# zhvng/open-musiclm

Measured on NVIDIA H100. Metric: coarse-stage training tokens/sec (positions fed to the transformer per optimiser step / step time), higher is better.
Workload: dtype bf16 (fp16 operands for the forward GEMMs on LayerNorm outputs x weights; fp32 accumulate)

## Files before the change

### open-musiclm_b200/csrc/gemm_tc.cu

```cuda
#include "common.cuh"
#include "ptx.cuh"
#include "../../include/omlm_b200.h"
#include <stdlib.h>
#include <algorithm>

namespace omlm {

constexpr int BM = 128;
constexpr int BK = 64;
constexpr int kGemmThreads = 384;

struct EpiParams {
  void* out;
  const float* addend;
  long ldo;
  long ldadd;
  float alpha;
  int out_f32;
  int atomic;
  long split_stride;
  int vec_ok;
  int row_split;
  int row_valid;
  int n_valid;
  const __nv_bfloat16* rs_hn;
  long rs_ldhn;
  const float* rs_gamma;
  const uint8_t* rs_keep;
  float2* rs_part;
  float rs_keep_scale;
  int rs_parts;
};

__device__ __forceinline__ float bf16lo(uint32_t v) { return __uint_as_float(v << 16); }
__device__ __forceinline__ float bf16hi(uint32_t v) { return __uint_as_float(v & 0xffff0000u); }

template <int BN>
struct GemmSmem {
  static constexpr int kABytes = BM * BK * 2;
  static constexpr int kBBytes = BN * BK * 2;
  static constexpr int kStageBytes = kABytes + kBBytes;
  static constexpr int kMaxStages = 8;
};

template <int BN, int A_MN, int B_MN, bool F16, bool RS = false>
__global__ void __launch_bounds__(kGemmThreads, 1)
gemm_bf16_kernel(const __grid_constant__ CUtensorMap tmA, const __grid_constant__ CUtensorMap tmB,
                 const EpiParams ep, const int M, const int N, const int K, const int splits, const int kStages) {
  using S = GemmSmem<BN>;
  extern __shared__ uint8_t smem_raw[];
  uint8_t* smem = smem_raw + ((1024u - (smem_u32(smem_raw) & 1023u)) & 1023u);
  uint64_t* full_bar = reinterpret_cast<uint64_t*>(smem + kStages * S::kStageBytes);
  uint64_t* empty_bar = full_bar + S::kMaxStages;

  const int wg = threadIdx.x >> 7;
  const int lane = threadIdx.x & 31;

  const int m_tiles = (M + BM - 1) / BM;
  const int n_tiles = (N + BN - 1) / BN;
  const int kb_total = (K + BK - 1) / BK;
  const int kb_per_split = (kb_total + splits - 1) / splits;
  const int tiles_total = m_tiles * n_tiles;
  const int work_total = tiles_total * splits;

  if (threadIdx.x == 0) {
    tma_prefetch_desc(&tmA);
    tma_prefetch_desc(&tmB);
    for (int i = 0; i < kStages; ++i) {
      mbar_init(&full_bar[i], 1);
      mbar_init(&empty_bar[i], 2);
    }
    fence_barrier_init();
  }
  __syncthreads();

  if (wg == 0) {
    asm volatile("setmaxnreg.dec.sync.aligned.u32 40;");
    if (threadIdx.x == 0) {
      int stage = 0;
      uint32_t phase = 0;
      for (int w = blockIdx.x; w < work_total; w += gridDim.x) {
        const int split = w / tiles_total;
        const int tile = w - split * tiles_total;
        const int n_blk = tile % n_tiles, m_blk = tile / n_tiles;
        const int kb0 = split * kb_per_split;
        const int kb1 = min(kb_total, kb0 + kb_per_split);
        for (int kb = kb0; kb < kb1; ++kb) {
          mbar_wait(&empty_bar[stage], phase ^ 1);
          uint8_t* sa = smem + stage * S::kStageBytes;
          uint8_t* sb = sa + S::kABytes;
          mbar_expect_tx(&full_bar[stage], S::kStageBytes);
          if (A_MN == 0) {
            tma_load_2d(sa, &tmA, &full_bar[stage], kb * BK, m_blk * BM);
          } else {
#pragma unroll
            for (int c = 0; c < BM / 64; ++c)
              tma_load_2d(sa + c * 8192, &tmA, &full_bar[stage], m_blk * BM + c * 64, kb * BK);
          }
          if (B_MN == 0) {
            tma_load_2d(sb, &tmB, &full_bar[stage], kb * BK, n_blk * BN);
          } else {
#pragma unroll
            for (int c = 0; c < BN / 64; ++c)
              tma_load_2d(sb + c * 8192, &tmB, &full_bar[stage], n_blk * BN + c * 64, kb * BK);
          }
          if (++stage == kStages) { stage = 0; phase ^= 1; }
        }
      }
    }
    return;
  }

  asm volatile("setmaxnreg.inc.sync.aligned.u32 232;");
  const int cw = wg - 1;
  const int wq = (threadIdx.x >> 5) & 3;
  const int qr = lane >> 2, qc = lane & 3;
  const bool leader = (threadIdx.x & 127) == 0;
  int stage = 0;
  uint32_t phase = 0;
  for (int w = blockIdx.x; w < work_total; w += gridDim.x) {
    const int split = w / tiles_total;
    const int tile = w - split * tiles_total;
    const int n_blk = tile % n_tiles, m_blk = tile / n_tiles;
    const int kb0 = split * kb_per_split;
    const int kb1 = min(kb_total, kb0 + kb_per_split);
    float acc[BN / 2];
#pragma unroll
    for (int i = 0; i < BN / 2; ++i) acc[i] = 0.f;
    int prev = -1;
    for (int kb = kb0; kb < kb1; ++kb) {
      mbar_wait(&full_bar[stage], phase);
      const uint32_t sa = smem_u32(smem + stage * S::kStageBytes) + cw * 8192;
      const uint32_t sb = smem_u32(smem + stage * S::kStageBytes + S::kABytes);
      wgmma_fence();
#pragma unroll
      for (int k = 0; k < BK / 16; ++k) {
        const uint64_t ad = A_MN ? make_smem_desc(sa + k * 2048, 8192, 1024) : make_smem_desc(sa + k * 32, 16, 1024);
        const uint64_t bd = B_MN ? make_smem_desc(sb + k * 2048, 8192, 1024) : make_smem_desc(sb + k * 32, 16, 1024);
        const uint32_t accum = (kb > kb0 || k > 0) ? 1u : 0u;
        Wgmma<BN, F16>::template ss<A_MN, B_MN>(acc, ad, bd, accum);
      }
      wgmma_commit();
      wgmma_wait<1>();
      if (prev >= 0 && leader) mbar_arrive(&empty_bar[prev]);
      prev = stage;
      if (++stage == kStages) { stage = 0; phase ^= 1; }
    }
    wgmma_wait<0>();
    wgmma_reg_fence(acc);
    if (prev >= 0 && leader) mbar_arrive(&empty_bar[prev]);

    int row_in[2];
    long orow[2], arow[2];
    bool row_ok[2];
#pragma unroll
    for (int hr = 0; hr < 2; ++hr) {
      int row = m_blk * BM + cw * 64 + wq * 16 + qr + hr * 8;
      row_in[hr] = row;
      row_ok[hr] = row < M;
      if (ep.row_split > 0) {
        const int half = row / ep.row_split, r = row - half * ep.row_split;
        row_ok[hr] = row_ok[hr] && r < ep.row_valid;
        row = half * ep.row_valid + r;
      } else if (ep.row_split < 0) {
        const int w256 = row & 255, ch = ((row >> 8) << 7) + (w256 & 127);
        row_ok[hr] = row_ok[hr] && ch < ep.row_valid;
        row = (w256 >> 7) * ep.row_valid + ch;
      }
      orow[hr] = static_cast<long>(row) * ep.ldo;
      arow[hr] = static_cast<long>(row) * ep.ldadd;
    }
    constexpr int kEpiBatch = RS ? 4 : 8;
    float rs1[2][2] = {{0.f, 0.f}, {0.f, 0.f}}, rs2[2][2] = {{0.f, 0.f}, {0.f, 0.f}};
#pragma unroll
    for (int i0 = 0; i0 < BN / 8; i0 += kEpiBatch) {
      float2 add[2][kEpiBatch], gam[kEpiBatch];
      uint32_t hv[2][kEpiBatch], keep[2][kEpiBatch];
#pragma unroll
      for (int j = 0; j < kEpiBatch; ++j) {
        const int col = n_blk * BN + 8 * (i0 + j) + 2 * qc;
        const bool c0_ok = col < ep.n_valid, c1_ok = col + 1 < ep.n_valid;
        if constexpr (RS) gam[j] = c0_ok ? __ldg(reinterpret_cast<const float2*>(ep.rs_gamma + col)) : make_float2(0.f, 0.f);
#pragma unroll
// ... 32 lines not shown
            rs2[hr][hf] = fmaf(v0, bf16lo(hv[hr][j]), rs2[hr][hf]);
            rs2[hr][hf] = fmaf(v1, bf16hi(hv[hr][j]), rs2[hr][hf]);
          }
          if (!RS && ep.addend != nullptr) { v0 += add[hr][j].x; v1 += add[hr][j].y; }
          if (ep.atomic) {
            float* op = reinterpret_cast<float*>(ep.out) + orow[hr] + col;
            if (pair) asm volatile("red.global.add.v2.f32 [%0], {%1, %2};" ::"l"(op), "f"(v0), "f"(v1) : "memory");
            else { atomicAdd(op, v0); if (col + 1 < ep.n_valid) atomicAdd(op + 1, v1); }
          } else if (ep.out_f32) {
            float* op = reinterpret_cast<float*>(ep.out) + split * ep.split_stride + orow[hr] + col;
            if (pair) *reinterpret_cast<float2*>(op) = make_float2(v0, v1);
            else { op[0] = v0; if (col + 1 < ep.n_valid) op[1] = v1; }
          } else {
            __nv_bfloat16* op = reinterpret_cast<__nv_bfloat16*>(ep.out) + orow[hr] + col;
            if (pair) *reinterpret_cast<uint32_t*>(op) = pack_bf16x2(v0, v1);
            else { op[0] = __float2bfloat16_rn(v0); if (col + 1 < ep.n_valid) op[1] = __float2bfloat16_rn(v1); }
          }
        }
      }
    }
    if constexpr (RS) {
#pragma unroll
      for (int hr = 0; hr < 2; ++hr)
#pragma unroll
        for (int hf = 0; hf < 2; ++hf) {
          float a1 = rs1[hr][hf], a2 = rs2[hr][hf];
          a1 += __shfl_xor_sync(0xffffffffu, a1, 1); a1 += __shfl_xor_sync(0xffffffffu, a1, 2);
          a2 += __shfl_xor_sync(0xffffffffu, a2, 1); a2 += __shfl_xor_sync(0xffffffffu, a2, 2);
          const int row = m_blk * BM + cw * 64 + wq * 16 + qr + hr * 8;
          if (qc == 0 && row < M) ep.rs_part[static_cast<long>(row) * ep.rs_parts + 2 * n_blk + hf] = make_float2(a1 * ep.rs_keep_scale, a2);
        }
    }
  }
}

constexpr int kMaxDynSmem = 232448;
constexpr int kBarrierBytes = 256;

template <int BN, int A_MN, int B_MN, bool RS = false>
static int launch_gemm(const CUtensorMap& tmA, const CUtensorMap& tmB, const EpiParams& ep, int M, int N, int K, int splits,
                       int max_ctas, int f16, cudaStream_t stream) {
  using S = GemmSmem<BN>;
  auto kern = f16 ? gemm_bf16_kernel<BN, A_MN, B_MN, true, RS> : gemm_bf16_kernel<BN, A_MN, B_MN, false, RS>;
  int stages = (kMaxDynSmem - 1024 - kBarrierBytes) / S::kStageBytes;
  if (stages > 6) stages = 6;
  const int smem_bytes = stages * S::kStageBytes + kBarrierBytes + 1024;
  static bool configured[2] = {false, false};
  if (!configured[f16]) {
    OMLM_CUDA(cudaFuncSetAttribute(kern, cudaFuncAttributeMaxDynamicSharedMemorySize, kMaxDynSmem));
    configured[f16] = true;
  }
  const int m_tiles = (M + BM - 1) / BM, n_tiles = (N + BN - 1) / BN;
  const int work = m_tiles * n_tiles * splits;
  int grid = num_sms();
  if (max_ctas > 0 && max_ctas < grid) grid = max_ctas;
  if (work < grid) grid = work;
  OMLM_KLAUNCH((kern), grid, kGemmThreads, smem_bytes, stream, tmA, tmB, ep, M, N, K, splits, stages);
  OMLM_LAUNCH_CHECK();
  return 0;
}

}

namespace omlm {
struct RowStatArgs { const void* hn; long ldhn; const void* keep_bits; const float* gamma; float keep_scale; float* part; int parts; };
}

static int gemm16_impl(const void* A, int a_f16, int a_mn_major, long lda, const void* B, int b_f16, int b_mn_major,
                       long ldb, int M, int N, int K, void* out, int out_f32, long ldo,
                       const float* addend, long ldadd, float alpha, int splits,
                       int row_split, int row_valid, int n_valid, int block_n, int max_ctas,
                       void* stream_, const omlm::RowStatArgs* rs, long split_stride = 0) {
  using namespace omlm;
  cudaStream_t stream = reinterpret_cast<cudaStream_t>(stream_);
  OMLM_CHECK_ARG(M > 0 && N > 0 && K > 0, "gemm: empty problem %d x %d x %d", M, N, K);
  OMLM_CHECK_ARG(block_n == 128 || block_n == 256, "gemm: block_n must be 128 or 256");
  OMLM_CHECK_ARG(splits >= 1, "gemm: splits must be >= 1");
  OMLM_CHECK_ARG((a_f16 != 0) == (b_f16 != 0), "gemm: both operands must have the same 16-bit format (one wgmma takes one operand format)");
  OMLM_CHECK_ARG(splits == 1 || (out_f32 && addend == nullptr), "gemm: split-K needs fp32 atomic output and no addend");
  OMLM_CHECK_ARG(split_stride == 0 || (out_f32 && addend == nullptr && rs == nullptr), "gemm: partial slices need fp32 output");
  if (n_valid <= 0 || n_valid > N) n_valid = N;
  {
    const int kb_total = (K + BK - 1) / BK;
    if (splits > kb_total) splits = kb_total;
    const int per = (kb_total + splits - 1) / splits;
    splits = (kb_total + per - 1) / per;
  }
  CUtensorMap tmA, tmB;
  int rc;
  if (a_mn_major == 0) rc = make_tmap_bf16_2d(&tmA, A, (uint64_t)K, (uint64_t)M, (uint64_t)lda * 2, 64, BM);
  else                 rc = make_tmap_bf16_2d(&tmA, A, (uint64_t)M, (uint64_t)K, (uint64_t)lda * 2, 64, 64);
  if (rc) return rc;
  if (b_mn_major == 0) rc = make_tmap_bf16_2d(&tmB, B, (uint64_t)K, (uint64_t)N, (uint64_t)ldb * 2, 64, block_n);
  else                 rc = make_tmap_bf16_2d(&tmB, B, (uint64_t)N, (uint64_t)K, (uint64_t)ldb * 2, 64, 64);
  if (rc) return rc;
  EpiParams ep;
  ep.out = out; ep.addend = addend; ep.ldo = ldo; ep.ldadd = ldadd; ep.alpha = alpha;
  ep.out_f32 = out_f32; ep.atomic = (splits > 1 && split_stride == 0) ? 1 : 0; ep.split_stride = split_stride;
  const long esz = out_f32 ? 4 : 2;
  ep.vec_ok = ((ldo * esz) % 16 == 0) && ((reinterpret_cast<uintptr_t>(out) & 15) == 0) &&
              (addend == nullptr || ((ldadd * 4) % 16 == 0 && (reinterpret_cast<uintptr_t>(addend) & 15) == 0));
  ep.row_split = row_split; ep.row_valid = row_valid; ep.n_valid = n_valid;
  ep.rs_hn = nullptr; ep.rs_ldhn = 0; ep.rs_gamma = nullptr; ep.rs_keep = nullptr; ep.rs_part = nullptr; ep.rs_keep_scale = 1.f;
  ep.rs_parts = 0;
  const int f16 = a_f16 ? 1 : 0;
  const int key = (block_n == 256 ? 4 : 0) | (a_mn_major ? 2 : 0) | (b_mn_major ? 1 : 0);
  if (rs != nullptr) {
    OMLM_CHECK_ARG(block_n == 256 && N % 256 == 0 && n_valid == N && !out_f32 && addend == nullptr && splits == 1 && row_split == 0 &&
                   ep.vec_ok && rs->parts == 2 * (N / 256) && rs->ldhn % 8 == 0,
                   "gemm row statistics: needs 256-wide tiles, N %% 256 == 0, a dense bf16 output and parts == N / 128");
    OMLM_CHECK_ARG(key == 5, "gemm row statistics: only the A K-major / B MN-major 256-wide instantiation exists");
    ep.rs_hn = reinterpret_cast<const __nv_bfloat16*>(rs->hn); ep.rs_ldhn = rs->ldhn;
    ep.rs_gamma = rs->gamma; ep.rs_keep = reinterpret_cast<const uint8_t*>(rs->keep_bits);
    ep.rs_part = reinterpret_cast<float2*>(rs->part); ep.rs_keep_scale = rs->keep_scale; ep.rs_parts = rs->parts;
    return launch_gemm<256, 0, 1, true>(tmA, tmB, ep, M, N, K, splits, max_ctas, f16, stream);
  }
  switch (key) {
    case 0: return launch_gemm<128, 0, 0>(tmA, tmB, ep, M, N, K, splits, max_ctas, f16, stream);
    case 1: return launch_gemm<128, 0, 1>(tmA, tmB, ep, M, N, K, splits, max_ctas, f16, stream);
    case 3: return launch_gemm<128, 1, 1>(tmA, tmB, ep, M, N, K, splits, max_ctas, f16, stream);
    case 4: return launch_gemm<256, 0, 0>(tmA, tmB, ep, M, N, K, splits, max_ctas, f16, stream);
    case 5: return launch_gemm<256, 0, 1>(tmA, tmB, ep, M, N, K, splits, max_ctas, f16, stream);
    case 7: return launch_gemm<256, 1, 1>(tmA, tmB, ep, M, N, K, splits, max_ctas, f16, stream);
    default:
      set_last_error("gemm: operand majors (a_mn=%d, b_mn=%d) not instantiated", a_mn_major, b_mn_major);
      return 1;
  }
}

extern "C" int omlm_gemm16(const void* A, int a_f16, int a_mn_major, long lda, const void* B, int b_f16, int b_mn_major,
                           long ldb, int M, int N, int K, void* out, int out_f32, long ldo,
                           const float* addend, long ldadd, float alpha, int splits,
                           int row_split, int row_valid, int n_valid, int block_n, int max_ctas,
                           void* stream_) {
  return gemm16_impl(A, a_f16, a_mn_major, lda, B, b_f16, b_mn_major, ldb, M, N, K, out, out_f32, ldo, addend, ldadd, alpha, splits,
                     row_split, row_valid, n_valid, block_n, max_ctas, stream_, nullptr);
}

namespace omlm {
__global__ void __launch_bounds__(256)
splitk_reduce_kernel(float* __restrict__ out, long ldo, const float* __restrict__ part, long slice, long ldp, int splits,
                     int rows_out, int n_valid) {
  const long total = static_cast<long>(rows_out) * n_valid;
  for (long i = blockIdx.x * static_cast<long>(blockDim.x) + threadIdx.x; i < total; i += static_cast<long>(gridDim.x) * blockDim.x) {
    const long r = i / n_valid, c = i - r * n_valid;
    float v = out[r * ldo + c];
    for (int s = 0; s < splits; ++s) v += part[s * slice + r * ldp + c];
    out[r * ldo + c] = v;
  }
}

static int gemm_rows_out(int M, int row_split, int row_valid) {
  if (row_split > 0) return (M + row_split - 1) / row_split * row_valid;
  if (row_split < 0) return 2 * row_valid;
  return M;
}
// ... 66 lines not shown
```

### open-musiclm_b200/engine.py

```python
import math
import os
import weakref
from typing import List, Optional

import torch

from . import lib

CE_IGNORE = -100


def _round_up(x, m):
    return (x + m - 1) // m * m


class _Plan:

    def __init__(self, eng: "Engine", B: int, n_tok: List[int], device):
        self.B = B
        self.n_tok = list(n_tok)
        S = len(n_tok)
        self.N = sum(n + 1 for n in n_tok)
        self.M = B * self.N
        self.pos0 = list(itertools_accumulate([0] + [n + 1 for n in n_tok[:-1]]))
# ... 275 lines not shown
            floats = max(floats, 4 * sms * max(d, 128),
                         8 * sms * 128,
                         B * ((N + 127) // 128) * 7 * self.F)
            ws["det_attn"] = lib.AttnBwdDetWorkspace(dev, B, N, self.h)
            self._det_attn.add(ws["det_attn"])
            shapes = [(cp, d) for cp in self.Cp] + [(d, self.F), (2 * self.F, d), (d, self.HD), (self.HD, d), (128, d)]
            need = max(48 * m * _round_up(n, 4) * 4 for m, n in shapes)
            ws["det_wgrad"] = torch.empty(min(need, self.DET_WGRAD_PART_BYTES) // 4, device=dev, dtype=torch.float32)
            if self.det_sumsq_part is None:
                self.det_sumsq_part = torch.empty(4 * sms, device=dev, dtype=torch.float64)
            if self.det_rows is None:
                self.det_rows = lib.embed_row_markers(self.table.numel() // d, dev)
        ws["det_part"] = torch.empty(floats, device=dev, dtype=torch.float32)
        ws["det_train"] = train

    _sms = None
    KB_COST_256 = 2.0 / 1.04

    @classmethod
    def _num_sms(cls):
        if cls._sms is None:
            cls._sms = lib.num_sms()
        return cls._sms

    @classmethod
    def _tile_cost(cls, m, n, kb, bn, splits, epi):
        sms = cls._num_sms()
        tiles = ((m + 127) // 128) * ((n + bn - 1) // bn)
        waves = (tiles * splits + sms - 1) // sms
        per_kb = 1.0 if bn == 128 else cls.KB_COST_256
        return waves * (((kb + splits - 1) // splits) * per_kb + epi * (bn / 128.0))

    @classmethod
    def _bn_for(cls, m, n, k):
        kb = (k + 63) // 64
        if n <= 128:
            return 128
        return min((128, 256), key=lambda bn: cls._tile_cost(m, n, kb, bn, 1, 6.0))

    @staticmethod
    def _bn(N):
        return 256 if N % 256 == 0 or N >= 2048 else 128

    def build_bias_table(self, ws, N):
        if self.bias_type == "continuous":
            self._relpos_table(ws, N)
        elif self.bias_type == "t5":
            w = self.pview["transformer.rel_pos_bias.relative_attention_bias.weight"]
            lib.sgemm_small(w, (1, 1), ws["ones"], (1, 1), ws["table"], (ws["table"].stride(0), 1), self.h, N, 1)

    def bias_table_backward(self, ws, N, det=False):
        if self.bias_type == "continuous":
            self._relpos_backward(ws, N, det)
        elif self.bias_type == "t5":
            gw = self.gview["transformer.rel_pos_bias.relative_attention_bias.weight"]
            lib.colsum(ws["dtable"], 1, ws["dtable"].stride(0), gw[0], N, self.h, accumulate=True)

    def _relpos_table(self, ws, N):
        pv, Hr, h = self.pview, self.Hr, self.h
        pre = "transformer.rel_pos_bias.net."
        lib.sgemm_small(ws["rp_in"], (1, 1), pv[pre + "0.0.weight"], (1, 1), ws["rp_a"][0], (Hr, 1), N, Hr, 1,
                        Z=ws["rp_z"][0], bias=pv[pre + "0.0.bias"], act=1)
        for j in (1, 2):
            lib.split3_bf16(ws["rp_a"][j - 1], ws["rp_a3"][j - 1])
            lib.gemm(ws["rp_a3"][j - 1], self.pk_rp[j - 1], ws["rp_z"][j], block_n=128)
            lib.bias_silu(ws["rp_z"][j], pv[f"{pre}{j}.0.bias"], ws["rp_a"][j])
        lib.sgemm_small(ws["rp_a"][2], (Hr, 1), pv[pre + "3.weight"], (1, Hr), ws["table"], (1, N), N, h, Hr, bias=pv[pre + "3.bias"])

    def forward_core(self, pl: _Plan, ws, src_row, key_mask, train: bool, groups_wanted=None, drop: bool = False, capture=None):
        self.refresh_packed()
        B, N, M, d, h, HD, F, Fp = pl.B, pl.N, pl.M, self.d, self.h, self.HD, self.F, self.Fp
        pv = self.pview
        x = ws["x"]
        lib.embed_gather(self.table, src_row, x[0], pl.src_row2)
        self.build_bias_table(ws, N)
        drop_p = self.drop_p if drop else 0.0
        f16 = self.a16 != torch.bfloat16
        dup = f16 and train
        for l in range(self.L):
            i = l if train else 0
            xa, xm, xo = (x[2 * l], x[2 * l + 1], x[2 * l + 2]) if train else (x[0], x[1], x[0])
            p, pk = f"transformer.layers.{l}.", self.pk[l]
            xn = ws["xn16"] if f16 else ws["xn"][i]
            lib.layernorm_fwd(xa, pv[p + "0.norm.gamma"], xn, ws["xraw"][i], ws["st_a"][i], ycopy=ws["xn"][i] if dup else None)
            lib.gemm(xn, pk["wq"], ws["q_raw"][i], block_n=self._bn_for(M, HD, d))
            lib.gemm(ws["xraw"][i], pk["wkv_b"], ws["kv_raw"][i], block_n=128)
            lib.qk_l2norm_fwd(ws["q_raw"][i], ws["kv_raw"][i], pv[p + "0.q_scale"], pv[p + "0.k_scale"], ws["qn"][i], ws["kvn"][i], h)
            if capture is not None:
                capture.after_kv(l, ws["kvn"][i])
            lib.attn_fwd_tc(ws["qn"][i], ws["kvn"][i], ws["table"], key_mask, ws["o"][i], ws["lse"][i], B, N, h)
            lib.gemm(ws["o"][i], pk["wo_b"], xm, addend=xa, block_n=self._bn_for(M, d, HD))
            xn2 = ws["xn2_16"] if f16 else ws["xn2"][i]
            lib.layernorm_fwd(xm, pv[p + self.ffk["g1"]], xn2, None, ws["st_f"][i], ycopy=ws["xn2"][i] if dup else None)
            lib.gemm_ffn_up(xn2, pk["w1"], pk["conv"], ws["u"][i], ws["h"], ws["rowsum"], N, Fp)
            if capture is not None:
                capture.after_u(l, ws["u"][i])
            hn = ws["hn16"] if f16 else ws["hn"][i]
            lib.ffn_norm_fwd(ws["h"], ws["rowsum"], pk["gin"], hn, ws["st_i"][i], F, Fp, drop_p, self.seed, l,
                             keep_bits=ws["keep"][i] if drop_p > 0 else None, hn_copy=ws["hn"][i] if dup else None)
            lib.gemm(hn, pk["w2"], xo, addend=xm, block_n=self._bn_for(M, d, Fp))
        x_last = x[2 * self.L] if train else x[0]
        xf = ws["xf16"] if f16 else ws["xf"]
        lib.layernorm_fwd(x_last, pv["transformer.norm.gamma"], xf, None, ws["st_o"], pl.dest_row, ycopy=ws["xf"] if dup else None)
        for gi, (s, qi, cnt, base) in enumerate(pl.groups):
            if groups_wanted is not None and s not in groups_wanted:
                continue
            rows = B * cnt
            lib.gemm(xf[base:base + rows], self.pk_logit[s][qi], ws["logits"][gi], block_n=128)

    def _wgrad(self, dy, x, gout, m, n, det_part=None, **kw):
        k = dy.shape[0]
        kb = (k + 63) // 64
        s_max = max(1, min(kb // 8, 48))
        if det_part is not None:
            rs, rv, nv = kw.get("row_split", 0), kw.get("row_valid", 0), kw.get("n_valid", 0) or n
            rows_out = (m + rs - 1) // rs * rv if rs > 0 else (2 * rv if rs < 0 else m)
            s_max = max(1, min(s_max, det_part.numel() // (rows_out * _round_up(nv, 4))))
        best = None
        for bn in (128, 256):
            for s in range(1, s_max + 1):
                c = self._tile_cost(m, n, kb, bn, s, 14.0 if s > 1 else 10.0)
                if best is None or c < best[0]:
                    best = (c, bn, s)
        _, bn, s = best
        if det_part is not None:
            lib.gemm_splitk_det(dy, x, gout, det_part, a_mn=True, b_mn=True, M=m, N=n, K=k, splits=s, block_n=bn,
                                max_ctas=self.bwd_max_ctas, **kw)
        elif s > 1:
            lib.gemm(dy, x, gout, a_mn=True, b_mn=True, M=m, N=n, K=k, splits=s, block_n=bn, max_ctas=self.bwd_max_ctas, **kw)
        else:
            lib.gemm(dy, x, gout, a_mn=True, b_mn=True, M=m, N=n, K=k, addend=gout, block_n=bn, max_ctas=self.bwd_max_ctas, **kw)

    def backward_core(self, pl: _Plan, ws, src_row, key_mask, groups_with_grad, drop: bool = False, on_ready=None, det: bool = False):
# ... 177 lines not shown
```

### open-musiclm_b200/csrc/attn_bwd_tc.cu

```cuda
#include "common.cuh"
#include "ptx.cuh"
#include "../../include/omlm_b200.h"
#include <stdlib.h>

namespace omlm {

constexpr int kBtThreads = 384;
constexpr int kBtBQ = 64, kBtBK = 128;
constexpr float kBtL2e = 1.4426950408889634f;

constexpr int kBoK = 0, kBoV = 16384, kBoQ = 32768 , kBoDO = 49152 ;
constexpr int kBoP = 65536 , kBoDS = 81920 , kBoBar = 98304 ;
constexpr int kBoSds = 98368;
constexpr int kBtMaxSmem = 232448;
constexpr int kBtSdsLd = 72;
constexpr int kBoWin = kBoSds + 2 * 64 * kBtSdsLd * 4;

static int bt_win_ld(int h) { return ((62 + h) / h + 64 + 23) / 32 * 32 + 8; }

__device__ __forceinline__ float bt_ex2(float x) {
  float y;
  asm("ex2.approx.ftz.f32 %0, %1;" : "=f"(y) : "f"(x));
  return y;
}
__device__ __forceinline__ void bt_red2(float* addr, float a, float b) {
  asm volatile("red.global.add.v2.f32 [%0], {%1, %2};" ::"l"(addr), "f"(a), "f"(b) : "memory");
}

__device__ __forceinline__ int bt_ld_acquire(const int* p) {
  int v;
  asm volatile("ld.acquire.gpu.global.b32 %0, [%1];" : "=r"(v) : "l"(p) : "memory");
  return v;
}
__device__ __forceinline__ unsigned long long bt_globaltimer() {
  unsigned long long t;
  asm volatile("mov.u64 %0, %%globaltimer;" : "=l"(t));
  return t;
}
__device__ __noinline__ void bt_wait_turn(const int* ctr, int turn, int* err) {
  const unsigned long long t0 = bt_globaltimer();
  while (bt_ld_acquire(ctr) != turn) {
    if (*reinterpret_cast<volatile int*>(err) != 0) return;
    if (bt_globaltimer() - t0 > 4000000000ull) { atomicExch(err, 1); return; }
    __nanosleep(64);
  }
}
__device__ __forceinline__ void bt_pass_turn(int* ctr) {
  asm volatile("red.release.gpu.global.add.s32 [%0], 1;" ::"l"(ctr) : "memory");
}

struct BtDet {
  int* turn_dq;
  int* turn_kv;
  int* meta;
  int* err;
  float* dpart;
};

template <bool DET>
// ... 46 lines not shown
      tma_load_2d(smem + kBoK, &tmKV, kv_full, 0, b * N + j0);
      tma_load_2d(smem + kBoV, &tmKV, kv_full, 64, b * N + j0);
      for (int t = 0; t < T; ++t) {
        const int st = t & 1;
        mbar_wait(&qd_empty[st], ((t >> 1) & 1) ^ 1);
        mbar_expect_tx(&qd_full[st], 2 * 8192);
        tma_load_2d(smem + kBoQ + st * 8192, &tmQ, &qd_full[st], 0, b * R + (rt0 + t) * kBtBQ);
        tma_load_2d(smem + kBoDO + st * 8192, &tmDO, &qd_full[st], 0, b * R + (rt0 + t) * kBtBQ);
      }
    }
  } else {
    asm volatile("setmaxnreg.inc.sync.aligned.u32 232;");
    const int cw = wg - 1;
    const int wq = (threadIdx.x >> 5) & 3, qr = lane >> 2, qc = lane & 3;
    const bool leader = (threadIdx.x & 127) == 0;
    const int kbase = j0 + cw * 64;
    const uint32_t sk = smem_u32(smem + kBoK) + cw * 8192, sv = smem_u32(smem + kBoV) + cw * 8192;
    uint8_t* p_tile = smem + kBoP + cw * 8192;
    uint8_t* ds_tile = smem + kBoDS + cw * 8192;
    float* sdsf = reinterpret_cast<float*>(smem + kBoSds) + cw * 64 * kBtSdsLd;
    float* win = reinterpret_cast<float*>(smem + kBoWin) + cw * h * win_ld;
    float* wacc = dacc + cw * h * Wacc;
    const int tid128 = threadIdx.x & 127;
    const uint32_t sp = smem_u32(p_tile), sds = smem_u32(ds_tile);
    const float sc2 = scale * kBtL2e;
    uint32_t vis = 0;
#pragma unroll
    for (int c = 0; c < 8; ++c)
#pragma unroll
      for (int e = 0; e < 2; ++e) {
        const int j = kbase + 8 * c + 2 * qc + e;
        if (j < N && (key_mask == nullptr || key_mask[static_cast<long long>(b) * N + j] != 0)) vis |= 1u << (2 * c + e);
      }
    float dv[32], dk[32];
#pragma unroll
    for (int x = 0; x < 32; ++x) { dv[x] = 0.f; dk[x] = 0.f; }
    mbar_wait(kv_full, 0);
    for (int t = 0; t < T; ++t) {
      const int st = t & 1;
      const int rbase = (rt0 + t) * kBtBQ;
      const uint32_t sq = smem_u32(smem + kBoQ + st * 8192), sdo = smem_u32(smem + kBoDO + st * 8192);
      mbar_wait(&qd_full[st], (t >> 1) & 1);
      float s[32], dp[32];
      wgmma_fence();
#pragma unroll
      for (int ks = 0; ks < 4; ++ks) {
        Wgmma<64, false>::ss<0, 0>(s, make_smem_desc(sq + ks * 32, 16, 1024), make_smem_desc(sk + ks * 32, 16, 1024), ks > 0 ? 1u : 0u);
        Wgmma<64, false>::ss<0, 0>(dp, make_smem_desc(sdo + ks * 32, 16, 1024), make_smem_desc(sv + ks * 32, 16, 1024), ks > 0 ? 1u : 0u);
      }
      wgmma_commit();
      const int it_lo = min(rbase, R - 1) / h, it_hi = min(rbase + kBtBQ - 1, R - 1) / h;
      {
        const int win_w = it_hi - it_lo + 64, dlo = it_lo - kbase - 63;
        for (int x = tid128; x < h * win_w; x += 128) {
          const int hh = x / win_w, w = x - hh * win_w, d = dlo + w;
          win[hh * win_ld + w] = d >= 0 ? __ldg(table + hh * static_cast<long>(table_ld) + d) * kBtL2e : 0.f;
        }
      }
      asm volatile("bar.sync %0, 128;" ::"r"(1 + cw) : "memory");
      wgmma_wait<0>();
      wgmma_reg_fence(s);
      wgmma_reg_fence(dp);
#pragma unroll
      for (int hr = 0; hr < 2; ++hr) {
        const int lr = wq * 16 + qr + hr * 8;
        const int r = rbase + lr;
        const bool row_ok = r < R;
        const int rc = min(r, R - 1);
        const int i = rc / h, hh = rc - i * h;
        const float lse = lse2[static_cast<long long>(b) * R + rc];
        const float D = dsum[static_cast<long long>(b) * R + rc];
        const float* wrow = win + hh * win_ld + i - it_lo + 63 - 2 * qc;
        const int dcol = i - kbase - 2 * qc;
        uint8_t* prow = p_tile + lr * 128;
        uint8_t* drow = ds_tile + lr * 128;
#pragma unroll
        for (int c = 0; c < 8; ++c) {
          float pp[2], dd[2];
#pragma unroll
          for (int e = 0; e < 2; ++e) {
            const bool live = row_ok && ((vis >> (2 * c + e)) & 1u) && dcol >= 8 * c + e;
            const float x = s[4 * c + 2 * hr + e];
            pp[e] = live ? bt_ex2(fmaf(x, sc2, wrow[-8 * c - e]) - lse) : 0.f;
            dd[e] = pp[e] * (dp[4 * c + 2 * hr + e] - D);
          }
          *reinterpret_cast<float2*>(sdsf + lr * kBtSdsLd + 8 * c + 2 * qc) = make_float2(dd[0], dd[1]);
          const uint32_t off = static_cast<uint32_t>(((c ^ (lr & 7)) << 4) + 4 * qc);
          *reinterpret_cast<uint32_t*>(prow + off) = pack_bf16x2(pp[0], pp[1]);
          *reinterpret_cast<uint32_t*>(drow + off) = pack_bf16x2(dd[0], dd[1]);
        }
      }
      fence_proxy_async();
      asm volatile("bar.sync %0, 128;" ::"r"(1 + cw) : "memory");
      float dq[32];
      wgmma_fence();
#pragma unroll
      for (int ks = 0; ks < 4; ++ks) {
        Wgmma<64, false>::ss<1, 1>(dv, make_smem_desc(sp + ks * 2048, 8192, 1024), make_smem_desc(sdo + ks * 2048, 8192, 1024), 1u);
        Wgmma<64, false>::ss<1, 1>(dk, make_smem_desc(sds + ks * 2048, 8192, 1024), make_smem_desc(sq + ks * 2048, 8192, 1024), 1u);
        Wgmma<64, false>::ss<0, 1>(dq, make_smem_desc(sds + ks * 32, 16, 1024), make_smem_desc(sk + ks * 2048, 8192, 1024), ks > 0 ? 1u : 0u);
      }
      wgmma_commit();
      {
        const int dlo = max(0, it_lo - kbase - 63), dhi = it_hi - kbase;
        const int W = dhi - dlo + 1;
        for (int p = tid128; p < h * W; p += 128) {
          const int hh = p / W, dl = dlo + (p - hh * W);
          const int i0 = max((rbase - hh + h - 1) / h, kbase + dl);
          const int i1 = min(min((rbase + kBtBQ - 1 - hh) / h, N - 1), kbase + dl + 63);
          float sum = 0.f;
          for (int i = i0; i <= i1; ++i) sum += sdsf[(i * h + hh - rbase) * kBtSdsLd + (i - dl - kbase)];
          wacc[hh * Wacc + dl - dmin] += sum;
        }
      }
      wgmma_wait<0>();
      wgmma_reg_fence(dq);
      wgmma_reg_fence(dv);
      wgmma_reg_fence(dk);
      asm volatile("bar.sync %0, 128;" ::"r"(1 + cw) : "memory");
      if (leader) mbar_arrive(&qd_empty[st]);
      int* turn = DET ? det.turn_dq + static_cast<long>(b) * n_rt + rt0 + t : nullptr;
      if constexpr (DET) {
        if (leader) bt_wait_turn(turn, 2 * kt + cw, det.err);
        asm volatile("bar.sync %0, 128;" ::"r"(1 + cw) : "memory");
      }
#pragma unroll
      for (int hr = 0; hr < 2; ++hr) {
        const int r = rbase + wq * 16 + qr + hr * 8;
        if (r < R) {
          float* dst = dqn + (static_cast<long long>(b) * R + r) * 64 + 2 * qc;
#pragma unroll
          for (int c = 0; c < 8; ++c) bt_red2(dst + 8 * c, dq[4 * c + 2 * hr] * scale, dq[4 * c + 2 * hr + 1] * scale);
        }
      }
      if constexpr (DET) {
        __threadfence();
        asm volatile("bar.sync %0, 128;" ::"r"(1 + cw) : "memory");
        if (leader) bt_pass_turn(turn);
      }
    }
    int* kv_turn = DET ? det.turn_kv + (static_cast<long>(b) * n_kt + kt) * 2 + cw : nullptr;
    if constexpr (DET) {
      if (leader) bt_wait_turn(kv_turn, u, det.err);
      asm volatile("bar.sync %0, 128;" ::"r"(1 + cw) : "memory");
    }
// ... 53 lines not shown
  const long tid = static_cast<long>(blockIdx.x) * blockDim.x + threadIdx.x;
  const long r = tid >> 3;
  const int sub = threadIdx.x & 7;
  float s = 0.f;
  for (long i = tid; i < kv_vec4; i += static_cast<long>(gridDim.x) * blockDim.x)
    reinterpret_cast<float4*>(dkvn)[i] = make_float4(0.f, 0.f, 0.f, 0.f);
  if (r < rows) {
    float4* zq = reinterpret_cast<float4*>(dqn + r * 64 + sub * 8);
    zq[0] = make_float4(0.f, 0.f, 0.f, 0.f);
    zq[1] = make_float4(0.f, 0.f, 0.f, 0.f);
    const uint4 a = *reinterpret_cast<const uint4*>(d_o + r * 64 + sub * 8);
    const uint4 bq = *reinterpret_cast<const uint4*>(o + r * 64 + sub * 8);
    const uint32_t aa[4] = {a.x, a.y, a.z, a.w}, bb[4] = {bq.x, bq.y, bq.z, bq.w};
#pragma unroll
    for (int i = 0; i < 4; ++i) {
      const float2 x = unpack_bf16x2(aa[i]), y = unpack_bf16x2(bb[i]);
      s += x.x * y.x + x.y * y.y;
    }
  }
  s += __shfl_xor_sync(0xffffffffu, s, 1);
  s += __shfl_xor_sync(0xffffffffu, s, 2);
  s += __shfl_xor_sync(0xffffffffu, s, 4);
  if (r < rows && sub == 0) dsum[r] = s;
}

}

namespace omlm {

struct BtConfig {
  int tiles_per_chunk, wacc, win_ld, smem_bytes, units_per_batch, n_row_tiles, n_key_tiles;
};

static int bt_config(int B, int N, int heads, BtConfig* cfg) {
  const long R = static_cast<long>(N) * heads;
  const int n_row_tiles = static_cast<int>((R + kBtBQ - 1) / kBtBQ);
  const int n_key_tiles = (N + kBtBK - 1) / kBtBK;
  const int win_ld = bt_win_ld(heads);
  auto wacc_of = [&](int T) { return (T * kBtBQ + heads - 1) / heads + kBtBK + 2; };
  auto smem_of = [&](int T) { return kBoWin + 2 * heads * (win_ld + wacc_of(T)) * 4 + 1024; };
  auto units_of = [&](int T) {
    long units = 0;
    for (int kt = 0; kt < n_key_tiles; ++kt) {
      const int first = (kt * kBtBK * heads) / kBtBQ;
      units += (n_row_tiles - first + T - 1) / T;
    }
    return units;
  };
  OMLM_CHECK_ARG(smem_of(1) <= kBtMaxSmem, "attn_bwd_tc: too many heads (%d) for the shared-memory bias tables", heads);
  int tiles_per_chunk = 1;
  for (int cand = 2; cand <= 2 * n_row_tiles; cand *= 2) {
    const int T = cand < n_row_tiles ? cand : n_row_tiles;
    if (smem_of(T) > kBtMaxSmem) break;
    tiles_per_chunk = T;
    if ((T >= 8 && units_of(T) * B <= 4L * num_sms()) || T == n_row_tiles) break;
  }
  if (const char* e = getenv("OMLM_ATTN_BWD_T")) {
    const int T = atoi(e);
    if (T >= 1 && T <= n_row_tiles && smem_of(T) <= kBtMaxSmem) tiles_per_chunk = T;
  }
  cfg->tiles_per_chunk = tiles_per_chunk;
  cfg->wacc = wacc_of(tiles_per_chunk);
  cfg->win_ld = win_ld;
  cfg->smem_bytes = smem_of(tiles_per_chunk);
  cfg->units_per_batch = static_cast<int>(units_of(tiles_per_chunk));
  cfg->n_row_tiles = n_row_tiles;
  cfg->n_key_tiles = n_key_tiles;
  return 0;
}

static int bt_ints(int B, const BtConfig& c) {
  return B * c.n_row_tiles + 2 * B * c.n_key_tiles + 2 * B * c.units_per_batch + 1;
}

static int attn_bwd_tc_impl(const void* qn, const void* kvn, const void* d_o, const void* o, const float* lse2,
                            const float* table, int table_ld, const unsigned char* key_mask, float* dsum_scratch,
                            float* dqn, float* dkvn, float* dtable, int B, int N, int heads, float scale, bool det,
                            float* ws, long ws_bytes, int* iws, long iws_count, void* stream) {
  OMLM_CHECK_ARG(B > 0 && N > 0 && heads > 0, "attn_bwd_tc: bad shape");
  OMLM_CHECK_ARG(table_ld >= N, "attn_bwd_tc: bias table shorter than the sequence");
  auto st = reinterpret_cast<cudaStream_t>(stream);
  const long R = static_cast<long>(N) * heads;
  const long rows = static_cast<long>(B) * R;
  BtConfig cfg;
  int rc = bt_config(B, N, heads, &cfg);
  if (rc) return rc;
  const int units = B * cfg.units_per_batch;
  BtDet dp{nullptr, nullptr, nullptr, nullptr, nullptr};
  if (det) {
// ... 67 lines not shown
```

Baseline: 726,700.

## Stage GEMM epilogue through shared memory with TMA stores and prefetched addend

Adds a staged epilogue to the warp-specialized GEMM. Accumulators are written into a swizzled shared-memory buffer and then stored with TMA. When a residual addend exists, a second producer warp prefetches it with TMA into that buffer, double-buffered per consumer warpgroup. This replaces uncoalesced per-thread global stores and loads, and also retunes block_n selection costs for residual GEMMs. In exchange the staging buffer takes shared memory from the pipeline, so fewer stages fit, and synchronization becomes more complex.

```diff
diff --git a/open-musiclm_b200/csrc/gemm_tc.cu b/open-musiclm_b200/csrc/gemm_tc.cu
--- a/open-musiclm_b200/csrc/gemm_tc.cu
+++ b/open-musiclm_b200/csrc/gemm_tc.cu
@@ -2,6 +2,7 @@
 #include "ptx.cuh"
 #include "../../include/omlm_b200.h"
 #include <stdlib.h>
+#include <string.h>
 #include <algorithm>
 
 namespace omlm {
@@ -20,6 +21,7 @@
   int atomic;
   long split_stride;
   int vec_ok;
+  int stg_bytes;
   int row_split;
   int row_valid;
   int n_valid;
@@ -43,15 +45,27 @@
   static constexpr int kMaxStages = 8;
 };
 
+__device__ __forceinline__ void named_bar_sync(int id, int threads) {
+  asm volatile("bar.sync %0, %1;" ::"r"(id), "r"(threads) : "memory");
+}
+
+constexpr int kStgChunk = 64 * 128;
+
 template <int BN, int A_MN, int B_MN, bool F16, bool RS = false>
 __global__ void __launch_bounds__(kGemmThreads, 1)
 gemm_bf16_kernel(const __grid_constant__ CUtensorMap tmA, const __grid_constant__ CUtensorMap tmB,
+                 const __grid_constant__ CUtensorMap tmO, const __grid_constant__ CUtensorMap tmAdd,
                  const EpiParams ep, const int M, const int N, const int K, const int splits, const int kStages) {
   using S = GemmSmem<BN>;
   extern __shared__ uint8_t smem_raw[];
   uint8_t* smem = smem_raw + ((1024u - (smem_u32(smem_raw) & 1023u)) & 1023u);
-  uint64_t* full_bar = reinterpret_cast<uint64_t*>(smem + kStages * S::kStageBytes);
+  uint8_t* stg = smem + kStages * S::kStageBytes;
+  const bool staged = !RS && ep.stg_bytes > 0;
+  const bool stg_add = staged && ep.addend != nullptr;
+  uint64_t* full_bar = reinterpret_cast<uint64_t*>(stg + ep.stg_bytes);
   uint64_t* empty_bar = full_bar + S::kMaxStages;
+  uint64_t* add_full = empty_bar + S::kMaxStages;
+  uint64_t* add_empty = add_full + 2;
 
   const int wg = threadIdx.x >> 7;
   const int lane = threadIdx.x & 31;
@@ -66,9 +80,15 @@
   if (threadIdx.x == 0) {
     tma_prefetch_desc(&tmA);
     tma_prefetch_desc(&tmB);
+    if (staged) tma_prefetch_desc(&tmO);
+    if (stg_add) tma_prefetch_desc(&tmAdd);
     for (int i = 0; i < kStages; ++i) {
       mbar_init(&full_bar[i], 1);
       mbar_init(&empty_bar[i], 2);
+    }
+    for (int h = 0; h < 2; ++h) {
+      mbar_init(&add_full[h], 1);
+      mbar_init(&add_empty[h], 1);
     }
     fence_barrier_init();
   }
@@ -107,6 +127,18 @@
           if (++stage == kStages) { stage = 0; phase ^= 1; }
         }
       }
+    } else if (threadIdx.x == 32 && stg_add) {
+      const int half = ep.stg_bytes / 2;
+      uint32_t j = 0;
+      for (int w = blockIdx.x; w < work_total; w += gridDim.x, ++j) {
+        const int n_blk = w % n_tiles, m_blk = w / n_tiles;
+        for (int h = 0; h < 2; ++h) {
+          mbar_wait(&add_empty[h], (j & 1) ^ 1);
+          mbar_expect_tx(&add_full[h], half);
+          for (int c = 0; c < half / kStgChunk; ++c)
+            tma_load_2d(stg + h * half + c * kStgChunk, &tmAdd, &add_full[h], n_blk * BN + c * 32, m_blk * BM + h * 64);
+        }
+      }
     }
     return;
   }
@@ -118,12 +150,14 @@
   const bool leader = (threadIdx.x & 127) == 0;
   int stage = 0;
   uint32_t phase = 0;
+  uint32_t add_phase = 0;
   for (int w = blockIdx.x; w < work_total; w += gridDim.x) {
     const int split = w / tiles_total;
     const int tile = w - split * tiles_total;
     const int n_blk = tile % n_tiles, m_blk = tile / n_tiles;
     const int kb0 = split * kb_per_split;
     const int kb1 = min(kb_total, kb0 + kb_per_split);
+    const bool free_stg = stg_add && leader && w != static_cast<int>(blockIdx.x);
     float acc[BN / 2];
 #pragma unroll
     for (int i = 0; i < BN / 2; ++i) acc[i] = 0.f;
@@ -141,6 +175,10 @@
         Wgmma<BN, F16>::template ss<A_MN, B_MN>(acc, ad, bd, accum);
       }
       wgmma_commit();
+      if (free_stg && kb == kb0) {
+        tma_store_wait_read<0>();
+        mbar_arrive(&add_empty[cw]);
+      }
       wgmma_wait<1>();
       if (prev >= 0 && leader) mbar_arrive(&empty_bar[prev]);
       prev = stage;
@@ -149,6 +187,43 @@
     wgmma_wait<0>();
     wgmma_reg_fence(acc);
     if (prev >= 0 && leader) mbar_arrive(&empty_bar[prev]);
+
+    if (staged) {
+      uint8_t* sbuf = stg + cw * (ep.stg_bytes / 2);
+      if (stg_add) {
+        mbar_wait(&add_full[cw], add_phase);
+        add_phase ^= 1;
+      } else {
+        if (leader) tma_store_wait_read<0>();
+        named_bar_sync(1 + cw, 128);
+      }
+      const int r = wq * 16 + qr;
+#pragma unroll
+      for (int i = 0; i < BN / 8; ++i) {
+#pragma unroll
+        for (int hr = 0; hr < 2; ++hr) {
+          float v0 = acc[4 * i + 2 * hr] * ep.alpha, v1 = acc[4 * i + 2 * hr + 1] * ep.alpha;
+          if (ep.out_f32) {
+            float2* p = reinterpret_cast<float2*>(sbuf + (i >> 2) * kStgChunk + (r + 8 * hr) * 128 +
+                                                  (((2 * (i & 3) + (qc >> 1)) ^ qr) << 4)) + (qc & 1);
+            if (stg_add) { const float2 a = *p; v0 += a.x; v1 += a.y; }
+            *p = make_float2(v0, v1);
+          } else {
+            *reinterpret_cast<uint32_t*>(sbuf + (i >> 3) * kStgChunk + (r + 8 * hr) * 128 + (((i & 7) ^ qr) << 4) + 4 * qc) =
+                pack_bf16x2(v0, v1);
+          }
+        }
+      }
+      fence_proxy_async();
+      named_bar_sync(1 + cw, 128);
+      if (leader) {
+        const int cols = ep.out_f32 ? 32 : 64;
+        for (int c = 0; c < ep.stg_bytes / 2 / kStgChunk; ++c)
+          tma_store_2d(&tmO, sbuf + c * kStgChunk, n_blk * BN + c * cols, m_blk * BM + cw * 64);
+        tma_store_commit();
+      }
+      continue;
+    }
 
     int row_in[2];
     long orow[2], arow[2];
@@ -247,19 +322,20 @@
         }
     }
   }
+  if (staged && leader) tma_store_wait_all();
 }
 
 constexpr int kMaxDynSmem = 232448;
 constexpr int kBarrierBytes = 256;
 
 template <int BN, int A_MN, int B_MN, bool RS = false>
-static int launch_gemm(const CUtensorMap& tmA, const CUtensorMap& tmB, const EpiParams& ep, int M, int N, int K, int splits,
-                       int max_ctas, int f16, cudaStream_t stream) {
+static int launch_gemm(const CUtensorMap& tmA, const CUtensorMap& tmB, const CUtensorMap& tmO, const CUtensorMap& tmAdd,
+                       const EpiParams& ep, int M, int N, int K, int splits, int max_ctas, int f16, cudaStream_t stream) {
   using S = GemmSmem<BN>;
   auto kern = f16 ? gemm_bf16_kernel<BN, A_MN, B_MN, true, RS> : gemm_bf16_kernel<BN, A_MN, B_MN, false, RS>;
-  int stages = (kMaxDynSmem - 1024 - kBarrierBytes) / S::kStageBytes;
+  int stages = (kMaxDynSmem - 1024 - kBarrierBytes - ep.stg_bytes) / S::kStageBytes;
   if (stages > 6) stages = 6;
-  const int smem_bytes = stages * S::kStageBytes + kBarrierBytes + 1024;
+  const int smem_bytes = stages * S::kStageBytes + ep.stg_bytes + kBarrierBytes + 1024;
   static bool configured[2] = {false, false};
   if (!configured[f16]) {
     OMLM_CUDA(cudaFuncSetAttribute(kern, cudaFuncAttributeMaxDynamicSharedMemorySize, kMaxDynSmem));
@@ -270,7 +346,7 @@
   int grid = num_sms();
   if (max_ctas > 0 && max_ctas < grid) grid = max_ctas;
   if (work < grid) grid = work;
-  OMLM_KLAUNCH((kern), grid, kGemmThreads, smem_bytes, stream, tmA, tmB, ep, M, N, K, splits, stages);
+  OMLM_KLAUNCH((kern), grid, kGemmThreads, smem_bytes, stream, tmA, tmB, tmO, tmAdd, ep, M, N, K, splits, stages);
   OMLM_LAUNCH_CHECK();
   return 0;
 }
@@ -316,6 +392,20 @@
   ep.vec_ok = ((ldo * esz) % 16 == 0) && ((reinterpret_cast<uintptr_t>(out) & 15) == 0) &&
               (addend == nullptr || ((ldadd * 4) % 16 == 0 && (reinterpret_cast<uintptr_t>(addend) & 15) == 0));
   ep.row_split = row_split; ep.row_valid = row_valid; ep.n_valid = n_valid;
+  CUtensorMap tmO, tmAdd;
+  memset(&tmO, 0, sizeof(tmO));
+  memset(&tmAdd, 0, sizeof(tmAdd));
+  ep.stg_bytes = 0;
+  if (rs == nullptr && splits == 1 && split_stride == 0 && row_split == 0 && ep.vec_ok && (n_valid * esz) % 16 == 0 &&
+      (addend == nullptr || out_f32) && !(block_n == 256 && out_f32)) {
+    ep.stg_bytes = static_cast<int>(BM * block_n * esz);
+    rc = make_tmap_2d(&tmO, static_cast<int>(esz), out, (uint64_t)n_valid, (uint64_t)M, (uint64_t)(ldo * esz), 128 / esz, 64);
+    if (rc) return rc;
+    if (addend != nullptr) {
+      rc = make_tmap_2d(&tmAdd, 4, addend, (uint64_t)n_valid, (uint64_t)M, (uint64_t)(ldadd * 4), 32, 64);
+      if (rc) return rc;
+    }
+  }
   ep.rs_hn = nullptr; ep.rs_ldhn = 0; ep.rs_gamma = nullptr; ep.rs_keep = nullptr; ep.rs_part = nullptr; ep.rs_keep_scale = 1.f;
   ep.rs_parts = 0;
   const int f16 = a_f16 ? 1 : 0;
@@ -328,15 +418,15 @@
     ep.rs_hn = reinterpret_cast<const __nv_bfloat16*>(rs->hn); ep.rs_ldhn = rs->ldhn;
     ep.rs_gamma = rs->gamma; ep.rs_keep = reinterpret_cast<const uint8_t*>(rs->keep_bits);
     ep.rs_part = reinterpret_cast<float2*>(rs->part); ep.rs_keep_scale = rs->keep_scale; ep.rs_parts = rs->parts;
-    return launch_gemm<256, 0, 1, true>(tmA, tmB, ep, M, N, K, splits, max_ctas, f16, stream);
+    return launch_gemm<256, 0, 1, true>(tmA, tmB, tmO, tmAdd, ep, M, N, K, splits, max_ctas, f16, stream);
   }
   switch (key) {
-    case 0: return launch_gemm<128, 0, 0>(tmA, tmB, ep, M, N, K, splits, max_ctas, f16, stream);
-    case 1: return launch_gemm<128, 0, 1>(tmA, tmB, ep, M, N, K, splits, max_ctas, f16, stream);
-    case 3: return launch_gemm<128, 1, 1>(tmA, tmB, ep, M, N, K, splits, max_ctas, f16, stream);
-    case 4: return launch_gemm<256, 0, 0>(tmA, tmB, ep, M, N, K, splits, max_ctas, f16, stream);
-    case 5: return launch_gemm<256, 0, 1>(tmA, tmB, ep, M, N, K, splits, max_ctas, f16, stream);
-    case 7: return launch_gemm<256, 1, 1>(tmA, tmB, ep, M, N, K, splits, max_ctas, f16, stream);
+    case 0: return launch_gemm<128, 0, 0>(tmA, tmB, tmO, tmAdd, ep, M, N, K, splits, max_ctas, f16, stream);
+    case 1: return launch_gemm<128, 0, 1>(tmA, tmB, tmO, tmAdd, ep, M, N, K, splits, max_ctas, f16, stream);
+    case 3: return launch_gemm<128, 1, 1>(tmA, tmB, tmO, tmAdd, ep, M, N, K, splits, max_ctas, f16, stream);
+    case 4: return launch_gemm<256, 0, 0>(tmA, tmB, tmO, tmAdd, ep, M, N, K, splits, max_ctas, f16, stream);
+    case 5: return launch_gemm<256, 0, 1>(tmA, tmB, tmO, tmAdd, ep, M, N, K, splits, max_ctas, f16, stream);
+    case 7: return launch_gemm<256, 1, 1>(tmA, tmB, tmO, tmAdd, ep, M, N, K, splits, max_ctas, f16, stream);
     default:
       set_last_error("gemm: operand majors (a_mn=%d, b_mn=%d) not instantiated", a_mn_major, b_mn_major);
       return 1;
diff --git a/open-musiclm_b200/engine.py b/open-musiclm_b200/engine.py
--- a/open-musiclm_b200/engine.py
+++ b/open-musiclm_b200/engine.py
@@ -331,11 +331,12 @@
         return waves * (((kb + splits - 1) // splits) * per_kb + epi * (bn / 128.0))
 
     @classmethod
-    def _bn_for(cls, m, n, k):
+    def _bn_for(cls, m, n, k, addend=False):
         kb = (k + 63) // 64
         if n <= 128:
             return 128
-        return min((128, 256), key=lambda bn: cls._tile_cost(m, n, kb, bn, 1, 6.0))
+        epi = {128: 8.0, 256: 13.0} if addend else {128: 1.0, 256: 1.0}
+        return min((128, 256), key=lambda bn: cls._tile_cost(m, n, kb, bn, 1, epi[bn]))
 
     @staticmethod
     def _bn(N):
@@ -388,7 +389,7 @@
             if capture is not None:
                 capture.after_kv(l, ws["kvn"][i])
             lib.attn_fwd_tc(ws["qn"][i], ws["kvn"][i], ws["table"], key_mask, ws["o"][i], ws["lse"][i], B, N, h)
-            lib.gemm(ws["o"][i], pk["wo_b"], xm, addend=xa, block_n=self._bn_for(M, d, HD))
+            lib.gemm(ws["o"][i], pk["wo_b"], xm, addend=xa, block_n=self._bn_for(M, d, HD, addend=True))
             xn2 = ws["xn2_16"] if f16 else ws["xn2"][i]
             lib.layernorm_fwd(xm, pv[p + self.ffk["g1"]], xn2, None, ws["st_f"][i], ycopy=ws["xn2"][i] if dup else None)
             lib.gemm_ffn_up(xn2, pk["w1"], pk["conv"], ws["u"][i], ws["h"], ws["rowsum"], N, Fp)
@@ -397,7 +398,7 @@
             hn = ws["hn16"] if f16 else ws["hn"][i]
             lib.ffn_norm_fwd(ws["h"], ws["rowsum"], pk["gin"], hn, ws["st_i"][i], F, Fp, drop_p, self.seed, l,
                              keep_bits=ws["keep"][i] if drop_p > 0 else None, hn_copy=ws["hn"][i] if dup else None)
-            lib.gemm(hn, pk["w2"], xo, addend=xm, block_n=self._bn_for(M, d, Fp))
+            lib.gemm(hn, pk["w2"], xo, addend=xm, block_n=self._bn_for(M, d, Fp, addend=True))
         x_last = x[2 * self.L] if train else x[0]
         xf = ws["xf16"] if f16 else ws["xf"]
         lib.layernorm_fwd(x_last, pv["transformer.norm.gamma"], xf, None, ws["st_o"], pl.dest_row, ycopy=ws["xf"] if dup else None)
```

Result: faster. 744,900, median of 6 (+2.5%).

## Prefetch bias window via cp.async, vectorize bias reduction, simulate chunk schedule

Applied to the files above, without the earlier changes.

Bias-table window loads and per-row lse/D loads for the next row tile are issued asynchronously with cp.async during the current tile's dQ/dK/dV MMAs, so their latency is hidden. The log2e scaling moves to the consumer. The relative-bias gradient reduction now unrolls eight rows at a time and uses incremental index stepping instead of per-element divisions. The tiles-per-chunk choice is replaced by a memoized greedy makespan simulation over SMs. In exchange the code gains more registers and host-side scheduling cost, and the cp.async window skips zero-filling entries with negative offsets.

```diff
diff --git a/open-musiclm_b200/csrc/attn_bwd_tc.cu b/open-musiclm_b200/csrc/attn_bwd_tc.cu
--- a/open-musiclm_b200/csrc/attn_bwd_tc.cu
+++ b/open-musiclm_b200/csrc/attn_bwd_tc.cu
@@ -2,6 +2,12 @@
 #include "ptx.cuh"
 #include "../../include/omlm_b200.h"
 #include <stdlib.h>
+#include <algorithm>
+#include <array>
+#include <functional>
+#include <map>
+#include <mutex>
+#include <vector>
 
 namespace omlm {
 
@@ -25,6 +31,9 @@
 }
 __device__ __forceinline__ void bt_red2(float* addr, float a, float b) {
   asm volatile("red.global.add.v2.f32 [%0], {%1, %2};" ::"l"(addr), "f"(a), "f"(b) : "memory");
+}
+__device__ __forceinline__ void bt_cp_async4(float* dst, const float* src) {
+  asm volatile("cp.async.ca.shared.global [%0], [%1], 4;" ::"r"(smem_u32(dst)), "l"(src) : "memory");
 }
 
 __device__ __forceinline__ int bt_ld_acquire(const int* p) {
@@ -137,6 +146,23 @@
         const int j = kbase + 8 * c + 2 * qc + e;
         if (j < N && (key_mask == nullptr || key_mask[static_cast<long long>(b) * N + j] != 0)) vis |= 1u << (2 * c + e);
       }
+    auto fetch_tile = [&](int rb, float (&lse)[2], float (&D)[2]) {
+      const int it_lo = min(rb, R - 1) / h, it_hi = min(rb + kBtBQ - 1, R - 1) / h;
+      const int win_w = it_hi - it_lo + 64, dlo = it_lo - kbase - 63;
+      for (int hh = tid128 / win_w, w = tid128 - hh * win_w; hh < h;) {
+        if (dlo + w >= 0) bt_cp_async4(win + hh * win_ld + w, table + hh * static_cast<long>(table_ld) + dlo + w);
+        for (w += 128; w >= win_w; ++hh) w -= win_w;
+      }
+      asm volatile("cp.async.commit_group;" ::: "memory");
+#pragma unroll
+      for (int hr = 0; hr < 2; ++hr) {
+        const int rc = min(rb + wq * 16 + qr + hr * 8, R - 1);
+        lse[hr] = lse2[static_cast<long long>(b) * R + rc];
+        D[hr] = dsum[static_cast<long long>(b) * R + rc];
+      }
+    };
+    float lse_t[2], D_t[2];
+    fetch_tile(rt0 * kBtBQ, lse_t, D_t);
     float dv[32], dk[32];
 #pragma unroll
     for (int x = 0; x < 32; ++x) { dv[x] = 0.f; dk[x] = 0.f; }
@@ -155,13 +181,7 @@
       }
       wgmma_commit();
       const int it_lo = min(rbase, R - 1) / h, it_hi = min(rbase + kBtBQ - 1, R - 1) / h;
-      {
-        const int win_w = it_hi - it_lo + 64, dlo = it_lo - kbase - 63;
-        for (int x = tid128; x < h * win_w; x += 128) {
-          const int hh = x / win_w, w = x - hh * win_w, d = dlo + w;
-          win[hh * win_ld + w] = d >= 0 ? __ldg(table + hh * static_cast<long>(table_ld) + d) * kBtL2e : 0.f;
-        }
-      }
+      asm volatile("cp.async.wait_all;" ::: "memory");
       asm volatile("bar.sync %0, 128;" ::"r"(1 + cw) : "memory");
       wgmma_wait<0>();
       wgmma_reg_fence(s);
@@ -173,12 +193,14 @@
         const bool row_ok = r < R;
         const int rc = min(r, R - 1);
         const int i = rc / h, hh = rc - i * h;
-        const float lse = lse2[static_cast<long long>(b) * R + rc];
-        const float D = dsum[static_cast<long long>(b) * R + rc];
+        const float lse = lse_t[hr], D = D_t[hr];
         const float* wrow = win + hh * win_ld + i - it_lo + 63 - 2 * qc;
         const int dcol = i - kbase - 2 * qc;
         uint8_t* prow = p_tile + lr * 128;
         uint8_t* drow = ds_tile + lr * 128;
+        float wv[16];
+#pragma unroll
+        for (int x = 0; x < 16; ++x) wv[x] = wrow[-8 * (x >> 1) - (x & 1)];
 #pragma unroll
         for (int c = 0; c < 8; ++c) {
           float pp[2], dd[2];
@@ -186,7 +208,7 @@
           for (int e = 0; e < 2; ++e) {
             const bool live = row_ok && ((vis >> (2 * c + e)) & 1u) && dcol >= 8 * c + e;
             const float x = s[4 * c + 2 * hr + e];
-            pp[e] = live ? bt_ex2(fmaf(x, sc2, wrow[-8 * c - e]) - lse) : 0.f;
+            pp[e] = live ? bt_ex2(fmaf(x, sc2, wv[2 * c + e] * kBtL2e) - lse) : 0.f;
             dd[e] = pp[e] * (dp[4 * c + 2 * hr + e] - D);
           }
           *reinterpret_cast<float2*>(sdsf + lr * kBtSdsLd + 8 * c + 2 * qc) = make_float2(dd[0], dd[1]);
@@ -197,6 +219,7 @@
       }
       fence_proxy_async();
       asm volatile("bar.sync %0, 128;" ::"r"(1 + cw) : "memory");
+      if (t + 1 < T) fetch_tile(rbase + kBtBQ, lse_t, D_t);
       float dq[32];
       wgmma_fence();
 #pragma unroll
@@ -209,13 +232,25 @@
       {
         const int dlo = max(0, it_lo - kbase - 63), dhi = it_hi - kbase;
         const int W = dhi - dlo + 1;
-        for (int p = tid128; p < h * W; p += 128) {
-          const int hh = p / W, dl = dlo + (p - hh * W);
-          const int i0 = max((rbase - hh + h - 1) / h, kbase + dl);
-          const int i1 = min(min((rbase + kBtBQ - 1 - hh) / h, N - 1), kbase + dl + 63);
+        const int q0 = rbase / h, r0 = rbase - q0 * h;
+        const int q1 = (rbase + kBtBQ - 1) / h, r1 = rbase + kBtBQ - 1 - q1 * h;
+        for (int hh = W > 0 ? tid128 / W : h, w = W > 0 ? tid128 - hh * W : 0; hh < h;) {
+          const int dl = dlo + w;
+          const int i0 = max(q0 + (hh < r0 ? 1 : 0), kbase + dl);
+          const int i1 = min(min(q1 - (hh > r1 ? 1 : 0), N - 1), kbase + dl + 63);
+          const float* src = sdsf + (i0 * h + hh - rbase) * kBtSdsLd + (i0 - dl - kbase);
+          const int stride = h * kBtSdsLd + 1;
           float sum = 0.f;
-          for (int i = i0; i <= i1; ++i) sum += sdsf[(i * h + hh - rbase) * kBtSdsLd + (i - dl - kbase)];
+          for (int i = i0; i <= i1; i += 8, src += 8 * stride) {
+            float x[8];
+#pragma unroll
+            for (int k = 0; k < 8; ++k) x[k] = i + k <= i1 ? src[k * stride] : 0.f;
+#pragma unroll
+            for (int k = 0; k < 8; ++k)
+              if (i + k <= i1) sum += x[k];
+          }
           wacc[hh * Wacc + dl - dmin] += sum;
+          for (w += 128; w >= W && hh < h; ++hh) w -= W;
         }
       }
       wgmma_wait<0>();
@@ -335,6 +370,39 @@
   int tiles_per_chunk, wacc, win_ld, smem_bytes, units_per_batch, n_row_tiles, n_key_tiles;
 };
 
+template <class Fits>
+static int bt_pick_chunk(int B, int n_row_tiles, int n_key_tiles, int heads, Fits fits) {
+  static std::mutex mu;
+  static std::map<std::array<int, 5>, int> memo;
+  const int sms = num_sms();
+  const std::array<int, 5> key{B, n_row_tiles, n_key_tiles, heads, sms};
+  std::lock_guard<std::mutex> lock(mu);
+  const auto hit = memo.find(key);
+  if (hit != memo.end()) return hit->second;
+  int best_T = 1;
+  long best = -1;
+  std::vector<long> busy(sms);
+  for (int T = 1; T <= std::min(16, n_row_tiles); ++T) {
+    if (!fits(T)) break;
+    std::fill(busy.begin(), busy.end(), 0L);
+    for (int kt = 0; kt < n_key_tiles; ++kt) {
+      const int first = (kt * kBtBK * heads) / kBtBQ;
+      for (int rt = first; rt < n_row_tiles; rt += T) {
+        const long cost = std::min(T, n_row_tiles - rt) + 1;
+        for (int b = 0; b < B; ++b) {
+          std::pop_heap(busy.begin(), busy.end(), std::greater<long>());
+          busy.back() += cost;
+          std::push_heap(busy.begin(), busy.end(), std::greater<long>());
+        }
+      }
+    }
+    const long makespan = *std::max_element(busy.begin(), busy.end());
+    if (best < 0 || makespan <= best) { best = makespan; best_T = T; }
+  }
+  memo[key] = best_T;
+  return best_T;
+}
+
 static int bt_config(int B, int N, int heads, BtConfig* cfg) {
   const long R = static_cast<long>(N) * heads;
   const int n_row_tiles = static_cast<int>((R + kBtBQ - 1) / kBtBQ);
@@ -351,13 +419,7 @@
     return units;
   };
   OMLM_CHECK_ARG(smem_of(1) <= kBtMaxSmem, "attn_bwd_tc: too many heads (%d) for the shared-memory bias tables", heads);
-  int tiles_per_chunk = 1;
-  for (int cand = 2; cand <= 2 * n_row_tiles; cand *= 2) {
-    const int T = cand < n_row_tiles ? cand : n_row_tiles;
-    if (smem_of(T) > kBtMaxSmem) break;
-    tiles_per_chunk = T;
-    if ((T >= 8 && units_of(T) * B <= 4L * num_sms()) || T == n_row_tiles) break;
-  }
+  int tiles_per_chunk = bt_pick_chunk(B, n_row_tiles, n_key_tiles, heads, [&](int T) { return smem_of(T) <= kBtMaxSmem; });
   if (const char* e = getenv("OMLM_ATTN_BWD_T")) {
     const int T = atoi(e);
     if (T >= 1 && T <= n_row_tiles && smem_of(T) <= kBtMaxSmem) tiles_per_chunk = T;
```

Measured after the change: 727,000 before, 757,600 after, median of 6. +4.2%, better.
